# itmo153277/JoshUpscale

Hardware: AMD Instinct MI355X
Metric: frames/sec 480x270->1920x1080 recurrent SR (higher is better)
Workload: dtype bf16

## Files before the change

### joshupscale_amd/csrc/c_api.cpp

```cpp

#include "joshupscale_amd.h"
#ifdef JU_TEST_HOOKS
#include "joshupscale_amd_test.h"
#endif

#include <cstdio>
#include <cstring>
#include <fstream>
#include <ios>
#include <new>
#include <stdexcept>
#include <string>
#include <vector>

#include "engine.h"
#include "fp8.h"
#include "graphics.h"
#include "log.h"
#include "model.h"
#include "tiled.h"

struct ju_runtime {
	std::unique_ptr<ju::Engine> engine;
};
// ... 707 lines not shown
		if (key == nullptr || value == nullptr) throw std::invalid_argument("ju_get_stat: null argument");
#ifndef JU_TEST_HOOKS
		if (std::strcmp(key, "scene_detector_runs") == 0) throw std::invalid_argument("unknown stat scene_detector_runs");
#endif
		*value = engineOf(const_cast<ju_runtime *>(runtime)).stat(key);
	});
}

#ifdef JU_TEST_HOOKS
int ju_debug_set(const char *key, int value) {
	return guarded([&] {
		const std::string k = key ? key : "";
		if (k == "tower_variant") ju::setTowerVariant(value);
		else if (k == "resident_fault") ju::setResidentFault(value);
		else if (k == "tower_fast") ju::setResidentTowerFast(value);
		else if (k == "res_block_plain") ju::setResBlockPlain(value);
		else if (k == "fp8_block_form") ju::setFp8BlockForm(value);
		else if (k == "pass_rerun") ju::setPassRerun(value);
		else if (k == "step_rerun") ju::setStepRerun(value);
		else if (k == "group_rerun") ju::setGroupRerun(value);
		else throw std::invalid_argument("unknown debug key " + k);
	});
}

namespace {
struct ConversionHook {
	const char *name, *family;
	bool (*admits)(const ju::YuvFormatInfo &);
	int ops;
	bool rowStrides;
// ... 524 lines not shown
```

### joshupscale_amd/csrc/engine.cpp

```cpp
#include "engine.h"

#include <cstdio>

#include <algorithm>
#include <atomic>
#include <cstdlib>
#include <cstring>
#include <memory>
#include <mutex>
#include <sstream>
#include <stdexcept>

#include "dev_switch.h"
#include "fp8.h"
#include "graphics.h"
#include "log.h"

namespace ju {

namespace {
thread_local int g_DryLaunches = 0;
}
bool launchesAreDry() { return g_DryLaunches > 0; }
DryLaunchScope::DryLaunchScope() { ++g_DryLaunches; }
// ... 1651 lines not shown

double Engine::stat(const std::string &key) const {
	if (key == "graph_replays") return static_cast<double>(m_GraphReplays);
	if (key == "eager_runs") return static_cast<double>(m_EagerRuns);
	if (key == "graph_captures") return static_cast<double>(m_InlineCaptures);
	if (key == "prepared_captures") return static_cast<double>(m_PreparedCaptures);
	if (key == "registered_pairs") return static_cast<double>(m_RegisteredPairs.size());
	if (key == "recurrent") return m_Config.recurrent() ? 1.0 : 0.0;
	if (key == "output_select") return static_cast<double>(m_Config.outputSelect);
	if (key == "resident_tower") return m_Resident ? 1.0 : 0.0;
	if (key == "resident_flow") return m_ResidentFlow ? 1.0 : 0.0;
	if (key == "tower_fast") {
		return (m_Resident && !m_Fp8Tower && residentTowerFast() && !m_Calibrate &&
		        residentTowerFastGeometry(m_Config.frameHeight, m_Config.frameWidth, m_ResGX, m_ResGY, m_ResRH)) ? 1.0 : 0.0;
	}
	if (key == "fallbacks") return static_cast<double>(m_Fallbacks);
	if (key == "lookahead_frames") return static_cast<double>(m_BatchFrames);
	if (key == "lookahead_host_frames") return static_cast<double>(m_BatchHostFrames);
	if (key == "hbd_from_state") return m_HbdFromState ? 1.0 : 0.0;
	if (key == "lookahead_yuv_frames") return static_cast<double>(m_BatchYuvFrames);
	if (key == "lookahead_max") return static_cast<double>(m_BatchMax);
	if (key == "source_scaled") return m_SrcScale.set() ? 1.0 : 0.0;
	if (key == "output_scaled") return m_OutScale.set() ? 1.0 : 0.0;
	if (key == "source_filter") return static_cast<double>(m_SrcScale.filter());
	if (key == "output_filter") return static_cast<double>(m_OutScale.filter());
	if (key == "source_mask") return m_MaskW != 0 ? 1.0 : 0.0;
	if (key == "source_stage_frames") return static_cast<double>(m_SourceFrames);
	if (key == "group_frames") return static_cast<double>(m_GroupFrames);
	if (key == "group_yuv_frames") return static_cast<double>(m_GroupYuvFrames);
	if (key == "scene_group") return m_SceneGroup ? 1.0 : 0.0;
// ... 30 lines not shown
```

### joshupscale_amd/csrc/kernels.h

```cpp
#pragma once

#include <hip/hip_runtime_api.h>

#include <cstddef>
#include <cstdint>
#include <mutex>
#include <stdexcept>
#include <string>
#include <vector>

#include "tile_geometry.h"

namespace ju {

enum DType : int { kF16 = 0, kBF16 = 1 };

inline std::size_t dtypeSize(DType) { return 2; }

class PlanLog {
public:
	void note(const std::string &line) {
		std::lock_guard<std::mutex> lock(m_Mutex);
		for (const std::string &l : m_Lines) {
			if (l == line) return;
// ... 182 lines not shown
	const std::uint8_t *frame;
	std::ptrdiff_t frameStride;
	void *state;
	std::uint8_t *outU8;
	std::ptrdiff_t outStride;
	const unsigned *sums;
};
bool residentTowerGeometry(int H, int W, int numCUs, int *GX, int *GY, int *RH);
std::size_t residentMailboxBytes(int GX, int GY, bool leaky = false);
bool residentTowerFastGeometry(int H, int W, int GX, int GY, int RH);
void setResBlockPlain(int on);
bool resBlockPlain();
void setResidentTowerFast(int on);
void setFp8BlockForm(int form);
bool residentTowerFast();
inline std::size_t residentCounterBytes(int GX, int GY) {
	return (static_cast<std::size_t>(GX) * GY * 2 * sizeof(unsigned) + 63) / 64 * 64;
}
void launchResidentTower(DType dt, const ResidentTowerParams &p, hipStream_t stream);

bool residentTowerM16();
void setTowerVariant(int variant);
int towerVariant();
void setResidentFault(int n);
int residentFaultForTests();

struct ResidentTower8Params {
	const void *in;
	void *out;
	const void *weights;
// ... 346 lines not shown
```

### joshupscale_amd/csrc/tower_kernels.hip

```cpp
#include "kernel_common.h"

namespace ju {

namespace {

constexpr int kTowerThreads = 256;
constexpr int kTowerWBytes = 9 * 64 * 64 * 2;
constexpr int kTowerTileBytes = 10 * 34 * 128;
constexpr int kTowerLds = kTowerWBytes + 2 * kTowerTileBytes;

__device__ __forceinline__ void glds16(const void *g, void *l) {
	__builtin_amdgcn_global_load_lds((const __attribute__((address_space(1))) void *)g,
	    (__attribute__((address_space(3))) void *)l, 16, 0, 0);
}

struct TowerParams {
	const void *in;
	const void *wgt;
	const float *bias;
	const void *res;
	void *out;
	int H, W, pitch;
	int tilesX, numTiles;
	int relu;
// ... 291 lines not shown
	if (rwv != 32) return false;
#endif
	const int np2 = rhv >> 1;
	for (int par = 0; par < 2; ++par) {
		const int first = par ? 1 : 2;
		int n = 0;
		for (int k = 0; k < 2; ++k) {
			const int u = first + 2 * k;
			if (u < np2 && 2 * u + 3 <= rhv) n = k + 1;
		}
		const int mine = (np2 - par + 1) >> 1;
		if (n != 2 || (mine != 3 && mine != 4)) return false;
	}
	return true;
}

struct ResidentParams {
	const void *in;
	int inPitch;
	int hasHead;
	void *out;
	const void *weights;
	const float *bias;
	uint4 *mail;
	unsigned *count;
	unsigned *error;
	unsigned long long *debug;
	int H, W, pitch;
	int GX, GY, RH;
	int nLayers;
// ... 2 lines not shown
	const float *tailB1;
	const void *tailW2;
	const float *tailB2;
	const std::uint8_t *frame;
	std::ptrdiff_t frameStride;
	void *state;
	std::uint8_t *outU8;
	std::ptrdiff_t outStride;
	const unsigned *sums;
};

typedef unsigned long long u64;
typedef __attribute__((address_space(1))) u64 gu64;
typedef __attribute__((address_space(1))) unsigned gu32;

template <typename T, int VARIANT, bool HEAD, bool TAIL = false, bool LEAKY = false, bool FAST = false>
__global__ __launch_bounds__(256, 1) void tower_resident_kernel(ResidentParams p) {
	static_assert(!FAST || ((VARIANT == 0 || VARIANT == 4) && (JU_FAST_PRERUN == 2 || JU_FAST_PRERUN == 3)), "the fast schedule is built for the product only");
	extern __shared__ __attribute__((aligned(16))) unsigned char smem[];
	constexpr bool kNoMfma = VARIANT == 2 || VARIANT == 3;
#ifdef JU_NOXCHG_DEV
	constexpr bool xchg = false;
#else
	constexpr bool xchg = !(VARIANT == 1 || VARIANT == 3);
#endif
	const int tid = threadIdx.x;
	const int wave = tid >> 6;
	const int lane = tid & 63;
	const int px = lane & 31;
	const int hh = lane >> 5;
	const int ch = wave & 1;
	const int rp = wave >> 1;
	int region;
// ... 123 lines not shown
			__builtin_amdgcn_sched_barrier(0);
			u64 t;
			asm volatile("s_memtime %0\n\ts_waitcnt lgkmcnt(0)" : "=s"(t)::"memory");
			__builtin_amdgcn_sched_barrier(0);
			return t;
		} else {
			return 0;
		}
	};
	constexpr int kOrder[12] = {4, 5, 6, 7, 0, 1, 2, 3, 8, 9, 10, 11};
	constexpr bool kPlain = VARIANT == 8;
	constexpr int kPreRun = kPlain ? 0 : FAST ? JU_FAST_PRERUN : JU_PRERUN;
	constexpr int kPreBefore = kPlain ? 0 : JU_PREBEFORE;
	TowerAcc accPre0[2], accPre1[2], accPre2[2];
	static_assert(kPreRun >= 0 && kPreRun <= 3, "at most three interior units per wave");
	Vec8<T> fb[2][4];
	auto issue = [&](unsigned rowAddr, int m, int set, int j) __attribute__((always_inline)) {
#if JU_TOWER_M16
		const int dx = m >> 2, ks32 = (m >> 1) & 1, ph = m & 1;
		const unsigned a = rowAddr + colBase[dx] + (((unsigned)(ks32 * 4 + (lane >> 4)) ^ colSwz[dx]) << 4);
		if (ph) {
			if (j == 0) asm volatile("ds_read_b128 %0, %1 offset:2048" : "=v"(fb[set][0]) : "v"(a));
			else if (j == 1) asm volatile("ds_read_b128 %0, %1 offset:6400" : "=v"(fb[set][1]) : "v"(a));
			else if (j == 2) asm volatile("ds_read_b128 %0, %1 offset:10752" : "=v"(fb[set][2]) : "v"(a));
			else asm volatile("ds_read_b128 %0, %1 offset:15104" : "=v"(fb[set][3]) : "v"(a));
			return;
		}
#else
		const int dx = m >> 2, ks = m & 3;
		const unsigned a = rowAddr + colBase[dx] + (((unsigned)(ks * 2 + hh) ^ colSwz[dx]) << 4);
#endif
		if (j == 0) asm volatile("ds_read_b128 %0, %1" : "=v"(fb[set][0]) : "v"(a));
		else if (j == 1) asm volatile("ds_read_b128 %0, %1 offset:4352" : "=v"(fb[set][1]) : "v"(a));
		else if (j == 2) asm volatile("ds_read_b128 %0, %1 offset:8704" : "=v"(fb[set][2]) : "v"(a));
		else asm volatile("ds_read_b128 %0, %1 offset:13056" : "=v"(fb[set][3]) : "v"(a));
	};
	const int np2 = rhv >> 1;
	const bool mySingle = (rhv & 1) && rp == (np2 & 1);
	const int preFirst = rp ? 1 : 2;
	int nPre = 0;
#pragma unroll
	for (int k = 0; k < kPreRun; ++k) {
		const int u = preFirst + 2 * k;
		if (u < np2 && 2 * u + 3 <= rhv) nPre = k + 1;
	}
	if constexpr (FAST && kPreRun == 3) {
		const int mine = (np2 - rp + 1) >> 1;
		nPre = nPre < mine - 1 ? nPre : mine - 1;
	}
	const int preEnd = preFirst + 2 * nPre;
	auto isPre = [&](int u) __attribute__((always_inline)) { return u >= preFirst && u < preEnd; };
	auto nextWhole = [&](int u) __attribute__((always_inline)) {
		int v = u + 2;
		if (isPre(v)) v = preEnd;
		return v < np2 ? v : -1;
	};
	const int firstWhole = isPre(rp) ? (preEnd < np2 ? preEnd : -1) : (rp < np2 ? rp : -1);
	const bool streamsInUnit = (firstWhole >= 0 || mySingle) && !kNoMfma && !kPlain;
	constexpr bool kDefer = FAST;
	const bool deferShape = residentFastShape(rhv, rwv);
	if constexpr (FAST) {
		if (!deferShape) {
			if (tid == 0) __hip_atomic_store((gu32 *)p.error, 0x6f0u, __ATOMIC_RELAXED, __HIP_MEMORY_SCOPE_SYSTEM);
			return;
		}
	}

#if JU_TOWER_M16
	const bool validLo = (lane & 15) < rwv, validHi = 16 + (lane & 15) < rwv;
	auto groupValid = [&](const int g) __attribute__((always_inline)) { return FAST || ((g >> 1) ? validHi : validLo); };
#else
	const bool lanesValid = px < rwv;
	auto groupValid = [&](const int) __attribute__((always_inline)) { return lanesValid; };
#endif
	typedef unsigned u32x4 __attribute__((ext_vector_type(4)));
	const __amdgpu_buffer_rsrc_t mailRsrc = __builtin_amdgcn_make_buffer_rsrc(
	    (void *)p.mail, 0, (int)((size_t)p.GX * p.GY * 2 * (LEAKY ? 2 : 1) * kResMailSlots * 16), 0x00020000);
	constexpr int kSc1 = 16;
	Vec4<T> rvNext[2][4];
	auto epiValue = [&](auto resTag, const TowerAcc &a, const int g, const Vec4<T> &rv, float(&v)[4]) __attribute__((always_inline)) {
#pragma unroll
		for (int i = 0; i < 4; ++i) v[i] = accElem(a, 4 * g + i);
		if constexpr (decltype(resTag)::value) {
#pragma unroll
			for (int i = 0; i < 4; ++i) v[i] += static_cast<float>(rv[i]);
		}
		if constexpr (VARIANT == 5 && !LEAKY) {
			if (groupValid(g)) {
#pragma unroll
				for (int i = 0; i < 4; ++i) calibMax = fmaxf(calibMax, v[i]);
			}
		}
	};
	auto epiStore = [&](auto outTag, const int row, const int g, float(&v)[4]) __attribute__((always_inline)) {
		constexpr int outOff = decltype(outTag)::value;
		if constexpr (LEAKY) {
#pragma unroll
			for (int i = 0; i < 4; ++i) v[i] = fmaxf(v[i], v[i] * p.slope);
			if constexpr (VARIANT == 5) {
#pragma unroll
				for (int i = 0; i < 4; ++i) calibMax = fmaxf(calibMax, fabsf(v[i]));
			}
			*reinterpret_cast<Vec4<T> *>(smem + outOff + row * kResRowBytes + outsw[g]) = pack4<T>(v[0], v[1], v[2], v[3]);
		} else {
			*reinterpret_cast<Vec4<T> *>(smem + outOff + row * kResRowBytes + outsw[g]) =
			    reluPacked<T>(pack4<T>(v[0], v[1], v[2], v[3]));
		}
	};
	auto unitSeg = [&](auto rowsTag, auto kindTag, auto resTag, auto inTag, auto outTag, TowerAcc(&acc)[2],
	                   const int layer, const int unit, const bool primed, const int nextUnit,
	                   const bool nextFinish, auto streamTag, auto defTag, TowerAcc(&dacc)[2], const int dunit,
	                   auto epiTag) __attribute__((always_inline)) {
		constexpr bool streamNext = decltype(streamTag)::value;
		constexpr bool DEF = decltype(defTag)::value;
		constexpr bool EPI = decltype(epiTag)::value;
		constexpr int ROWS = decltype(rowsTag)::value;
		constexpr int KIND = decltype(kindTag)::value;
		constexpr bool residual = decltype(resTag)::value;
		constexpr int inOff = decltype(inTag)::value;
		constexpr int outOff = decltype(outTag)::value;
		constexpr int P0 = KIND == 1 ? 4 : 0;
		constexpr int P1 = KIND == 0 ? 4 : 12;
		const u64 tu0 = stamp();
		constexpr int NR = ROWS + 2;
		constexpr int NM = 3 * ROWS;
		const int ra = 1 + 2 * unit;
		if constexpr (KIND != 1 && kNoMfma) {
#pragma unroll
			for (int r = 0; r < ROWS; ++r) acc[r] = biasVec;
		}
		unsigned rowAddr = ldsBase + inOff + (2 * unit) * kResRowBytes;
		asm volatile("" : "+v"(rowAddr));
		constexpr bool kFetchRes = !EPI && residual && KIND != 0;
		const int dra = 1 + 2 * dunit;
		const TowerAcc dacc0 = dacc[0], dacc1 = dacc[1];
		float dv[4];
		unsigned dlo = 0, dhi = 0;
		auto defSlot = [&](const int pos, const int k, const int part = -1) __attribute__((always_inline)) {
					if constexpr (DEF) {
						const int j = pos - P0;
						if (j < 8) {
							const int r = j >> 2, g = j & 3;
							if (k < 5 && part == 1) {
							} else if (k < 4) {
								dv[k] = accElem(r ? dacc1 : dacc0, 4 * g + k);
								if constexpr (residual) {
									dv[k] += static_cast<float>(rvNext[r][g][k]);
									asm volatile("" : "+v"(dv[k]));
								}
								if constexpr (LEAKY) {
									const float t = dv[k] * p.slope;
									asm volatile("v_max_f32 %0, %1, %2" : "=v"(dv[k]) : "v"(dv[k]), "v"(t));
								}
							} else if (k == 4) {
								const Vec4<T> pk = pack4<T>(dv[0], dv[1], dv[2], dv[3]);
								typedef unsigned u32x2d __attribute__((ext_vector_type(2)));
								const u32x2d w = __builtin_bit_cast(u32x2d, pk);
								dlo = w[0];
								dhi = w[1];
								asm volatile("" : "+v"(dlo), "+v"(dhi));
							} else {
								typedef unsigned u32x2d __attribute__((ext_vector_type(2)));
								if (part != 1) {
									const Vec4<T> pk = __builtin_bit_cast(Vec4<T>, u32x2d{dlo, dhi});
									const u32x2d w = __builtin_bit_cast(u32x2d, LEAKY ? pk : reluPacked<T>(pk));
									dlo = w[0];
									dhi = w[1];
									if (part == 0) asm volatile("" : "+v"(dlo), "+v"(dhi));
								}
								if (part != 0) {
									const Vec4<T> o = __builtin_bit_cast(Vec4<T>, u32x2d{dlo, dhi});
									if (groupValid(g)) *reinterpret_cast<Vec4<T> *>(smem + outOff + (dra + r) * kResRowBytes + outsw[g]) = o;
								}
							}
						}
					}
		};
		if (!kNoMfma) {
			if (!primed) {
				asm volatile("s_waitcnt lgkmcnt(0)" ::: "memory");
				__builtin_amdgcn_sched_barrier(0);
#pragma unroll
				for (int j = 0; j < NR; ++j) issue(rowAddr, kOrder[P0], 0, j);
			}
#pragma unroll
			for (int pos = P0; pos < P1; ++pos) {
				const int m = kOrder[pos];
				const int set = (pos - P0) & 1;
				const bool more = (pos + 1 < P1);
				const int dx = m >> 2;
				[[maybe_unused]] const int ks = m & 3;
#pragma unroll
				for (int k = 0; k < NM; ++k) {
					const int dy = ROWS == 2 ? (k >> 1) : k;
					const int r = ROWS == 2 ? (k & 1) : 0;
					const int need = r + dy;
					const bool fresh = ROWS == 2 ? (k == 0 || k == 1 || k == 3 || k == 5) : true;
					if (fresh) {
						const int issuedNext = more ? (k < NR ? k : NR) : 0;
						const int younger = (DEF && pos > P0 && pos - P0 <= 8 ? 1 : 0) +
						                    (kFetchRes && pos == P1 - 1 ? 2 * (k < 4 ? k : 4) : 0);
						const int allowed = (NR - 1 - need) + issuedNext + younger;
						if (allowed >= 12) asm volatile("s_waitcnt lgkmcnt(12)" ::: "memory");
						else if (allowed == 11) asm volatile("s_waitcnt lgkmcnt(11)" ::: "memory");
						else if (allowed == 10) asm volatile("s_waitcnt lgkmcnt(10)" ::: "memory");
						else if (allowed == 9) asm volatile("s_waitcnt lgkmcnt(9)" ::: "memory");
						else if (allowed == 8) asm volatile("s_waitcnt lgkmcnt(8)" ::: "memory");
						else if (allowed == 7) asm volatile("s_waitcnt lgkmcnt(7)" ::: "memory");
						else if (allowed == 6) asm volatile("s_waitcnt lgkmcnt(6)" ::: "memory");
						else if (allowed == 5) asm volatile("s_waitcnt lgkmcnt(5)" ::: "memory");
						else if (allowed == 4) asm volatile("s_waitcnt lgkmcnt(4)" ::: "memory");
						else if (allowed == 3) asm volatile("s_waitcnt lgkmcnt(3)" ::: "memory");
						else if (allowed == 2) asm volatile("s_waitcnt lgkmcnt(2)" ::: "memory");
						else if (allowed == 1) asm volatile("s_waitcnt lgkmcnt(1)" ::: "memory");
						else asm volatile("s_waitcnt lgkmcnt(0)" ::: "memory");
						__builtin_amdgcn_sched_barrier(0);
					}
#if JU_TOWER_M16
					{
						const int ks32 = (m >> 1) & 1, ph = m & 1;
						const bool first = KIND != 1 && (pos == P0 || pos == P0 + 1) && dy == 0;
#pragma unroll
						for (int c16 = 0; c16 < 2; ++c16) {
							const int kf = ks32 * 2 + c16, sl = ph * 2 + c16;
							acc[r].q[sl] = mfma16(dx == 1 ? wm[dy * 4 + kf] : ws[dy * 8 + (dx >> 1) * 4 + kf], fb[set][need],
							    first ? biasVec.q[sl] : acc[r].q[sl]);
							if (c16 == 0) {
								defSlot(pos, k, 0);
								__builtin_amdgcn_sched_barrier(0);
							}
						}
						defSlot(pos, k, 1);
						if constexpr (KIND == 2) {
							if (streamNext && (m & 1) && (ROWS == 2 ? (k & 1) : true)) {
								const int sdy = ROWS == 2 ? (k >> 1) : k;
#pragma unroll
								for (int c16 = 0; c16 < 2; ++c16) {
									const int kf = ks32 * 2 + c16;
									const Vec8<T> nf = loadWeightFrag(layer + 1, (sdy * 3 + dx) * 4 + kf);
									if (dx == 1) wm[sdy * 4 + kf] = nf;
									else ws[sdy * 8 + (dx >> 1) * 4 + kf] = nf;
								}
							}
						}
					}
#else
					acc[r] = mfma32(dx == 1 ? wm[dy * 4 + ks] : ws[dy * 8 + (dx >> 1) * 4 + ks], fb[set][need],
					    (KIND != 1 && pos == P0 && dy == 0) ? biasVec : acc[r]);
#endif
					if (more && k < NR) issue(rowAddr, kOrder[pos + 1 < 12 ? pos + 1 : 11], set ^ 1, k);
#if !JU_TOWER_M16
					defSlot(pos, k);
#endif
					if constexpr (kFetchRes) {
						if (pos == P1 - 1 && k < 4) {
							const int ra0 = 1 + 2 * unit;
							rvNext[(2 * k) >> 2][(2 * k) & 3] = *reinterpret_cast<const Vec4<T> *>(
							    smem + outOff + (ra0 + ((2 * k) >> 2)) * kResRowBytes + outsw[(2 * k) & 3]);
							rvNext[(2 * k + 1) >> 2][(2 * k + 1) & 3] = *reinterpret_cast<const Vec4<T> *>(
							    smem + outOff + (ra0 + ((2 * k + 1) >> 2)) * kResRowBytes + outsw[(2 * k + 1) & 3]);
						}
					}
					__builtin_amdgcn_sched_barrier(0);
				}
				if constexpr (KIND == 2) {
					if (streamNext) {
#if JU_TOWER_M16
						if (pos == 1) loadBias(layer + 1);
#else
						if (pos == 0) loadBias(layer + 1);
// ... 2 lines not shown
#else
#pragma unroll
						for (int dy = 0; dy < 3; ++dy) {
							const Vec8<T> nf = loadWeightFrag(layer + 1, (dy * 3 + dx) * 4 + ks);
							if (dx == 1) wm[dy * 4 + ks] = nf;
							else ws[dy * 8 + (dx >> 1) * 4 + ks] = nf;
						}
#endif
						__builtin_amdgcn_sched_barrier(0);
					}
				}
			}
			if (nextUnit >= 0) {
				const unsigned na = ldsBase + inOff + (2 * nextUnit) * kResRowBytes;
				const bool nextSingle = (nextUnit == np2);
				if (nextFinish) {
#pragma unroll
					for (int j = 0; j < 4; ++j) issue(na, kOrder[4], 0, j);
				} else {
#pragma unroll
					for (int j = 0; j < 3; ++j) issue(na, kOrder[0], 0, j);
					if (!nextSingle) issue(na, kOrder[0], 0, 3);
				}
				__builtin_amdgcn_sched_barrier(0);
			}
		}
		const u64 tu1 = stamp();
		if constexpr (KIND == 0) prof[7] += tu1 - tu0;
#ifdef JU_TOWER_SEGPROF
		else if constexpr (KIND == 1 && !DEF) prof[3] += tu1 - tu0;
		else if constexpr (KIND == 1 && DEF) prof[4] += tu1 - tu0;
		else if constexpr (KIND == 2 && !streamNext) prof[5] += tu1 - tu0;
		else prof[6] += tu1 - tu0;
#else
		else prof[5] += tu1 - tu0;
#endif
		if constexpr (KIND != 0 && EPI) {
			{
				Vec4<T> rv[ROWS][4];
				if (residual) {
#pragma unroll
					for (int r = 0; r < ROWS; ++r) {
#pragma unroll
						for (int g = 0; g < 4; ++g) {
							rv[r][g] = *reinterpret_cast<const Vec4<T> *>(
							    smem + outOff + (ra + r) * kResRowBytes + outsw[g]);
						}
					}
					asm volatile("s_waitcnt lgkmcnt(0)" ::: "memory");
				}
#pragma unroll
				for (int r = 0; r < ROWS; ++r) {
// ... 4 lines not shown
						if (groupValid(g)) epiStore(outTag, ra + r, g, v);
					}
				}
			}
			const u64 tu2 = stamp();
#ifndef JU_TOWER_SEGPROF
			prof[6] += tu2 - tu1;
#endif
		}
	};
	using R2 = std::integral_constant<int, 2>;
	using R1 = std::integral_constant<int, 1>;
	using KPre = std::integral_constant<int, 0>;
	using KFin = std::integral_constant<int, 1>;
	using KWhole = std::integral_constant<int, 2>;
	auto preRun = [&](auto inTag, auto outTag, auto loTag, auto hiTag, const int layer, const bool primedFirst)
	                  __attribute__((always_inline)) {
		constexpr int LO = decltype(loTag)::value, HI = decltype(hiTag)::value;
		auto slot = [&](TowerAcc(&acc)[2], const int k) __attribute__((always_inline)) {
			if (k < nPre) {
				const int nu = (k + 1 < kPreRun && k + 1 < nPre) ? preFirst + 2 * (k + 1) : -1;
				unitSeg(R2{}, KPre{}, std::false_type{}, inTag, outTag, acc, layer, preFirst + 2 * k,
				    (k > 0 || primedFirst) && !kNoMfma, nu, false, std::false_type{}, std::false_type{}, acc, 0, std::true_type{});
			}
		};
		if constexpr (LO <= 0 && 0 < HI) slot(accPre0, 0);
		if constexpr (LO <= 1 && 1 < HI) slot(accPre1, 1);
		if constexpr (LO <= 2 && 2 < HI) slot(accPre2, 2);
	};
	auto finishLayer = [&](auto resTag, auto inTag, auto outTag, const int layer, const bool streamW) __attribute__((always_inline)) {
		const int afterPre = firstWhole >= 0 ? firstWhole : (mySingle ? np2 : -1);
		if constexpr (kDefer) {
			{
				using Y = std::true_type;
				using N = std::false_type;
				const int ua = firstWhole, ub = nextWhole(firstWhole);
				int lastUnit = ua;
				unitSeg(R2{}, KFin{}, resTag, inTag, outTag, accPre0, layer, preFirst, false, preFirst + 2, true, N{}, N{}, accPre0, 0, N{});
				if (kPreRun == 3 && nPre == 3) {
					unitSeg(R2{}, KFin{}, resTag, inTag, outTag, accPre1, layer, preFirst + 2, true, preFirst + 4, true, N{}, Y{}, accPre0, preFirst, N{});
					unitSeg(R2{}, KFin{}, resTag, inTag, outTag, accPre2, layer, preFirst + 4, true, ua, false, N{}, Y{}, accPre1, preFirst + 2, N{});
					if (streamW) unitSeg(R2{}, KWhole{}, resTag, inTag, outTag, accPre0, layer, ua, true, -1, false, Y{}, Y{}, accPre2, preFirst + 4, N{});
					else unitSeg(R2{}, KWhole{}, resTag, inTag, outTag, accPre0, layer, ua, true, -1, false, N{}, Y{}, accPre2, preFirst + 4, N{});
				} else {
					unitSeg(R2{}, KFin{}, resTag, inTag, outTag, accPre1, layer, preFirst + 2, true, ua, false, N{}, Y{}, accPre0, preFirst, N{});
					if (ub >= 0) {
						unitSeg(R2{}, KWhole{}, resTag, inTag, outTag, accPre2, layer, ua, true, ub, false, N{}, Y{}, accPre1, preFirst + 2, N{});
// ... 310 lines not shown
		if constexpr (VARIANT == 5) {
			float m = calibMax;
#pragma unroll
			for (int off = 32; off > 0; off >>= 1) m = fmaxf(m, __shfl_xor(m, off));
			if (lane == 0) atomicMax(reinterpret_cast<unsigned *>(p.debug) + i, __float_as_uint(m));
			calibMax = 0.f;
		}
		const u64 t1 = stamp();
		__syncthreads();
		const u64 t2 = stamp();
		if (more && xchg) publish(OutT{}, i);
		const bool primePre = more && nPre > 0 && !kNoMfma;
		if (primePre) {
			const unsigned na = ldsBase + OutT::value + (2 * preFirst) * kResRowBytes;
#pragma unroll
			for (int j = 0; j < 4; ++j) issue(na, kOrder[0], 0, j);
			__builtin_amdgcn_sched_barrier(0);
		}
		const u64 t3 = stamp();
		if (more && !streamsInUnit) {
			loadBias(i + 1);
			loadMidWeights(i + 1);
			loadSideWeights(i + 1);
		}
		const u64 t4 = stamp();
		if (more && xchg) {
			using Z = std::integral_constant<int, 0>;
			using Split = std::integral_constant<int, kPreBefore>;
			using N = std::integral_constant<int, kPreRun>;
			preRun(OutT{}, InT{}, Z{}, Split{}, i + 1, primePre);
			const bool okFill = fillHalo(OutT{}, i, [&]() __attribute__((always_inline)) {
// ... 85 lines not shown
		for (int i = tid; i < rhv * kResRW * 8; i += 256) {
			const int c = i & 7;
			const int pxl = (i >> 3) % kResRW;
			const int row = (i >> 3) / kResRW;
			if (pxl < rwv) {
				const int rr = row + 1, cc = pxl + 1;
				const uint4 v = *reinterpret_cast<const uint4 *>(
				    smem + finalOff + rr * kResRowBytes + cc * 128 + ((c ^ ((cc >> 1) & 7)) << 4));
				*reinterpret_cast<uint4 *>(
				    out + ((size_t)(y0 + rr) * p.pitch + x0 + cc) * 64 + c * 8) = v;
			}
		}
	}
}

template <typename T, int VARIANT, bool HEAD, bool TAIL = false, bool LEAKY = false, bool FAST = false>
void launchResidentT(const ResidentParams &p, hipStream_t stream) {
	auto kern = tower_resident_kernel<T, VARIANT, HEAD, TAIL, LEAKY, FAST>;
	static std::atomic<std::uint64_t> ldsDone{0};
	ensureDynamicLds(reinterpret_cast<const void *>(kern), kResLds, &ldsDone, "resident tower");
	const int grid = p.GX * p.GY - (g_ResidentFault < p.GX * p.GY ? g_ResidentFault : 0);
	hipLaunchKernelGGL(kern, dim3(grid), dim3(256), kResLds, stream, p);
	hipCheckLaunch("tower_resident");
}

}

void launchConvTower(DType dt, const ConvParams &p, hipStream_t stream) {
	const int pitch = towerPitch(p.W);
	const bool fits = p.taps == 9 && p.cin == 64 && p.cout == 64 && !p.outHead && p.nb == 2 &&
	                  p.inPitch == pitch && p.outPitch == pitch &&
	                  (p.res == nullptr || p.resPitch == pitch);
	if (!fits) {
// ... 24 lines not shown

bool residentTowerGeometry(int H, int W, int numCUs, int *GX, int *GY, int *RH) {
	const int gx = (W + kResRW - 1) / kResRW;
	const int gy = (H + kResMaxRH - 1) / kResMaxRH;
	if (gx * gy > numCUs) return false;
	*GX = gx;
	*GY = gy;
	*RH = (H + gy - 1) / gy;
	return true;
}

bool residentTowerFastGeometry(int H, int W, int GX, int GY, int RH) {
	const int lastH = H - (GY - 1) * RH, lastW = W - (GX - 1) * kResRW;
	return residentFastShape(RH, kResRW) && residentFastShape(lastH, kResRW) && residentFastShape(RH, lastW) &&
	       residentFastShape(lastH, lastW);
}

std::size_t residentMailboxBytes(int GX, int GY, bool leaky) {
	return static_cast<std::size_t>(GX) * GY * 2 * kResMailSlots * 16 * (leaky ? 2 : 1);
}

void launchResidentTower(DType dt, const ResidentTowerParams &q, hipStream_t stream) {
	ResidentParams p{};
	const std::size_t origin = towerOrigin(q.W) * 64 * 2;
	p.in = q.in;
	p.inPitch = q.inPitch ? q.inPitch : q.W;
	p.hasHead = q.hasHead;
	p.out = static_cast<unsigned char *>(q.out) - origin;
	p.weights = q.weights;
	p.bias = q.bias;
// ... 11 lines not shown
	p.slope = q.slope;
	p.tailW1 = q.tailW1;
	p.tailB1 = q.tailB1;
	p.tailW2 = q.tailW2;
	p.tailB2 = q.tailB2;
	p.frame = q.frame;
	p.frameStride = q.frameStride;
	p.state = q.state;
	p.outU8 = q.outU8;
	p.outStride = q.outStride;
	p.sums = q.sums;
	if ((p.nLayers & 1) != (p.hasHead ? 1 : 0)) {
		throw std::invalid_argument("resident tower: layer count must be 2*blocks (+1 with a head)");
	}
	const bool fast = residentTowerFast() && residentTowerFastGeometry(p.H, p.W, p.GX, p.GY, p.RH);
#ifdef JU_TOWER_DEV
	if (q.leaky || dt == kF16 || !p.hasHead) throw std::invalid_argument("resident tower: developer build");
	if (p.tailW1 != nullptr) {
		if (fast) launchResidentT<bf16, 0, true, true, false, true>(p, stream);
		else launchResidentT<bf16, 0, true, true>(p, stream);
	} else if (g_TowerVariant == 8) launchResidentT<bf16, 8, true>(p, stream);
	else if (g_TowerVariant == 4) {
		if (fast) launchResidentT<bf16, 4, true, false, false, true>(p, stream);
		else launchResidentT<bf16, 4, true>(p, stream);
	} else if (fast) launchResidentT<bf16, 0, true, false, false, true>(p, stream);
	else launchResidentT<bf16, 0, true>(p, stream);
	return;
#else
	if (q.leaky) {
		if (!(q.slope >= 0.0f && q.slope <= 1.0f)) throw std::invalid_argument("resident tower: negative slope outside [0, 1]");
		if (p.tailW1 != nullptr) throw std::invalid_argument("resident tower: the fused tail is built for ReLU models");
		if (!p.hasHead) {
			if (fast) {
				if (dt == kF16) launchResidentT<f16, 0, false, false, true, true>(p, stream);
				else launchResidentT<bf16, 0, false, false, true, true>(p, stream);
			} else {
				if (dt == kF16) launchResidentT<f16, 0, false, false, true>(p, stream);
				else launchResidentT<bf16, 0, false, false, true>(p, stream);
			}
		} else if (g_TowerVariant == 8) {
// ... 10 lines not shown
			else launchResidentT<bf16, 0, true, false, true>(p, stream);
		}
		return;
	}
	if (!p.hasHead) {
		if (fast) {
			if (dt == kF16) launchResidentT<f16, 0, false, false, false, true>(p, stream);
			else launchResidentT<bf16, 0, false, false, false, true>(p, stream);
		} else {
			if (dt == kF16) launchResidentT<f16, 0, false>(p, stream);
			else launchResidentT<bf16, 0, false>(p, stream);
		}
		return;
	}
	if (p.tailW1 != nullptr) {
		if (fast) {
			if (dt == kF16) launchResidentT<f16, 0, true, true, false, true>(p, stream);
			else launchResidentT<bf16, 0, true, true, false, true>(p, stream);
		} else {
			if (dt == kF16) launchResidentT<f16, 0, true, true>(p, stream);
			else launchResidentT<bf16, 0, true, true>(p, stream);
		}
		return;
	}
	if (dt == kF16) {
		if (g_TowerVariant == 8) launchResidentT<f16, 8, true>(p, stream);
		else if (fast) launchResidentT<f16, 0, true, false, false, true>(p, stream);
		else launchResidentT<f16, 0, true>(p, stream);
		return;
	}
	switch (g_TowerVariant) {
	case 8: launchResidentT<bf16, 8, true>(p, stream); break;
	case 1: launchResidentT<bf16, 1, true>(p, stream); break;
	case 2: launchResidentT<bf16, 2, true>(p, stream); break;
	case 3: launchResidentT<bf16, 3, true>(p, stream); break;
	case 4:
		if (fast) launchResidentT<bf16, 4, true, false, false, true>(p, stream);
		else launchResidentT<bf16, 4, true>(p, stream);
		break;
	case 5:
		(void)hipMemsetAsync(p.debug, 0, static_cast<std::size_t>(p.nLayers) * sizeof(unsigned), stream);
		launchResidentT<bf16, 5, true>(p, stream);
		break;
	default:
		if (fast) launchResidentT<bf16, 0, true, false, false, true>(p, stream);
		else launchResidentT<bf16, 0, true>(p, stream);
		break;
	}
#endif
}


}
```

Baseline: 2214.

## Process four output rows per unit in the fast resident tower schedule

Adds a UROWS=4 form of the resident tower kernel, where each MFMA unit computes four output rows instead of two. Each LDS input row fragment is then reused across more rows, and there are fewer unit segments per layer. The pre-run, finish and whole-unit segments, the deferred epilogue slots and the LDS-wait accounting are reworked for quads. It becomes the default when the tile geometry gives 14- or 16-row by 32-column tiles. In exchange it holds more accumulators and fragment registers, with extra register pressure and more complex scheduling.

Result: faster. 2246 (median of 6 runs) (+1.5%).

```diff
diff --git a/joshupscale_amd/csrc/c_api.cpp b/joshupscale_amd/csrc/c_api.cpp
--- a/joshupscale_amd/csrc/c_api.cpp
+++ b/joshupscale_amd/csrc/c_api.cpp
@@ -745,6 +745,7 @@
 		if (k == "tower_variant") ju::setTowerVariant(value);
 		else if (k == "resident_fault") ju::setResidentFault(value);
 		else if (k == "tower_fast") ju::setResidentTowerFast(value);
+		else if (k == "tower_unit_rows") ju::setResidentTowerUnitRows(value);
 		else if (k == "res_block_plain") ju::setResBlockPlain(value);
 		else if (k == "fp8_block_form") ju::setFp8BlockForm(value);
 		else if (k == "pass_rerun") ju::setPassRerun(value);
diff --git a/joshupscale_amd/csrc/engine.cpp b/joshupscale_amd/csrc/engine.cpp
--- a/joshupscale_amd/csrc/engine.cpp
+++ b/joshupscale_amd/csrc/engine.cpp
@@ -1689,6 +1689,10 @@
 		return (m_Resident && !m_Fp8Tower && residentTowerFast() && !m_Calibrate &&
 		        residentTowerFastGeometry(m_Config.frameHeight, m_Config.frameWidth, m_ResGX, m_ResGY, m_ResRH)) ? 1.0 : 0.0;
 	}
+	if (key == "tower_unit_rows") {
+		const bool fast = stat("tower_fast") != 0.0;
+		return (fast && m_Config.genActivation != 1) ? static_cast<double>(residentTowerUnitRows(m_Config.frameHeight, m_Config.frameWidth, m_ResGX, m_ResGY, m_ResRH)) : 2.0;
+	}
 	if (key == "fallbacks") return static_cast<double>(m_Fallbacks);
 	if (key == "lookahead_frames") return static_cast<double>(m_BatchFrames);
 	if (key == "lookahead_host_frames") return static_cast<double>(m_BatchHostFrames);
diff --git a/joshupscale_amd/csrc/kernels.h b/joshupscale_amd/csrc/kernels.h
--- a/joshupscale_amd/csrc/kernels.h
+++ b/joshupscale_amd/csrc/kernels.h
@@ -220,6 +220,8 @@
 void setResidentTowerFast(int on);
 void setFp8BlockForm(int form);
 bool residentTowerFast();
+int residentTowerUnitRows(int H, int W, int GX, int GY, int RH);
+void setResidentTowerUnitRows(int rows);
 inline std::size_t residentCounterBytes(int GX, int GY) {
 	return (static_cast<std::size_t>(GX) * GY * 2 * sizeof(unsigned) + 63) / 64 * 64;
 }
diff --git a/joshupscale_amd/csrc/tower_kernels.hip b/joshupscale_amd/csrc/tower_kernels.hip
--- a/joshupscale_amd/csrc/tower_kernels.hip
+++ b/joshupscale_amd/csrc/tower_kernels.hip
@@ -329,6 +329,8 @@
 	}
 	return true;
 }
+
+__host__ __device__ inline bool residentFastQuadShape(int rhv, int rwv) { return rwv == 32 && (rhv == 16 || rhv == 14); }
 
 struct ResidentParams {
 	const void *in;
@@ -361,9 +363,11 @@
 typedef __attribute__((address_space(1))) u64 gu64;
 typedef __attribute__((address_space(1))) unsigned gu32;
 
-template <typename T, int VARIANT, bool HEAD, bool TAIL = false, bool LEAKY = false, bool FAST = false>
+template <typename T, int VARIANT, bool HEAD, bool TAIL = false, bool LEAKY = false, bool FAST = false, int UROWS = 2>
 __global__ __launch_bounds__(256, 1) void tower_resident_kernel(ResidentParams p) {
 	static_assert(!FAST || ((VARIANT == 0 || VARIANT == 4) && (JU_FAST_PRERUN == 2 || JU_FAST_PRERUN == 3)), "the fast schedule is built for the product only");
+	static_assert(UROWS == 2 || (UROWS == 4 && FAST && !LEAKY && JU_TOWER_M16 && JU_FAST_PRERUN == 2 && JU_PREBEFORE == 1),
+	    "row quads are a form of the ReLU fast schedule in the 16x16x32 shape");
 	extern __shared__ __attribute__((aligned(16))) unsigned char smem[];
 	constexpr bool kNoMfma = VARIANT == 2 || VARIANT == 3;
 #ifdef JU_NOXCHG_DEV
@@ -517,7 +521,8 @@
 	constexpr int kPreBefore = kPlain ? 0 : JU_PREBEFORE;
 	TowerAcc accPre0[2], accPre1[2], accPre2[2];
 	static_assert(kPreRun >= 0 && kPreRun <= 3, "at most three interior units per wave");
-	Vec8<T> fb[2][4];
+	TowerAcc accQ0[4], accQ1[4];
+	Vec8<T> fb[2][UROWS + 2];
 	auto issue = [&](unsigned rowAddr, int m, int set, int j) __attribute__((always_inline)) {
 #if JU_TOWER_M16
 		const int dx = m >> 2, ks32 = (m >> 1) & 1, ph = m & 1;
@@ -526,7 +531,11 @@
 			if (j == 0) asm volatile("ds_read_b128 %0, %1 offset:2048" : "=v"(fb[set][0]) : "v"(a));
 			else if (j == 1) asm volatile("ds_read_b128 %0, %1 offset:6400" : "=v"(fb[set][1]) : "v"(a));
 			else if (j == 2) asm volatile("ds_read_b128 %0, %1 offset:10752" : "=v"(fb[set][2]) : "v"(a));
-			else asm volatile("ds_read_b128 %0, %1 offset:15104" : "=v"(fb[set][3]) : "v"(a));
+			else if (j == 3) asm volatile("ds_read_b128 %0, %1 offset:15104" : "=v"(fb[set][3]) : "v"(a));
+			else if constexpr (UROWS == 4) {
+				if (j == 4) asm volatile("ds_read_b128 %0, %1 offset:19456" : "=v"(fb[set][4]) : "v"(a));
+				else asm volatile("ds_read_b128 %0, %1 offset:23808" : "=v"(fb[set][5]) : "v"(a));
+			}
 			return;
 		}
 #else
@@ -536,17 +545,22 @@
 		if (j == 0) asm volatile("ds_read_b128 %0, %1" : "=v"(fb[set][0]) : "v"(a));
 		else if (j == 1) asm volatile("ds_read_b128 %0, %1 offset:4352" : "=v"(fb[set][1]) : "v"(a));
 		else if (j == 2) asm volatile("ds_read_b128 %0, %1 offset:8704" : "=v"(fb[set][2]) : "v"(a));
-		else asm volatile("ds_read_b128 %0, %1 offset:13056" : "=v"(fb[set][3]) : "v"(a));
+		else if (j == 3) asm volatile("ds_read_b128 %0, %1 offset:13056" : "=v"(fb[set][3]) : "v"(a));
+		else if constexpr (UROWS == 4) {
+			if (j == 4) asm volatile("ds_read_b128 %0, %1 offset:17408" : "=v"(fb[set][4]) : "v"(a));
+			else asm volatile("ds_read_b128 %0, %1 offset:21760" : "=v"(fb[set][5]) : "v"(a));
+		}
 	};
 	const int np2 = rhv >> 1;
 	const bool mySingle = (rhv & 1) && rp == (np2 & 1);
-	const int preFirst = rp ? 1 : 2;
+	const int preFirst = UROWS == 4 ? (rp ? 2 : 4) : (rp ? 1 : 2);
 	int nPre = 0;
 #pragma unroll
 	for (int k = 0; k < kPreRun; ++k) {
 		const int u = preFirst + 2 * k;
 		if (u < np2 && 2 * u + 3 <= rhv) nPre = k + 1;
 	}
+	if constexpr (UROWS == 4) nPre = 1;
 	if constexpr (FAST && kPreRun == 3) {
 		const int mine = (np2 - rp + 1) >> 1;
 		nPre = nPre < mine - 1 ? nPre : mine - 1;
@@ -559,9 +573,9 @@
 		return v < np2 ? v : -1;
 	};
 	const int firstWhole = isPre(rp) ? (preEnd < np2 ? preEnd : -1) : (rp < np2 ? rp : -1);
-	const bool streamsInUnit = (firstWhole >= 0 || mySingle) && !kNoMfma && !kPlain;
+	const bool streamsInUnit = UROWS == 4 || ((firstWhole >= 0 || mySingle) && !kNoMfma && !kPlain);
 	constexpr bool kDefer = FAST;
-	const bool deferShape = residentFastShape(rhv, rwv);
+	const bool deferShape = UROWS == 4 ? residentFastQuadShape(rhv, rwv) : residentFastShape(rhv, rwv);
 	if constexpr (FAST) {
 		if (!deferShape) {
 			if (tid == 0) __hip_atomic_store((gu32 *)p.error, 0x6f0u, __ATOMIC_RELAXED, __HIP_MEMORY_SCOPE_SYSTEM);
@@ -580,7 +594,7 @@
 	const __amdgpu_buffer_rsrc_t mailRsrc = __builtin_amdgcn_make_buffer_rsrc(
 	    (void *)p.mail, 0, (int)((size_t)p.GX * p.GY * 2 * (LEAKY ? 2 : 1) * kResMailSlots * 16), 0x00020000);
 	constexpr int kSc1 = 16;
-	Vec4<T> rvNext[2][4];
+	Vec4<T> rvNext[UROWS][4];
 	auto epiValue = [&](auto resTag, const TowerAcc &a, const int g, const Vec4<T> &rv, float(&v)[4]) __attribute__((always_inline)) {
 #pragma unroll
 		for (int i = 0; i < 4; ++i) v[i] = accElem(a, 4 * g + i);
@@ -610,10 +624,10 @@
 			    reluPacked<T>(pack4<T>(v[0], v[1], v[2], v[3]));
 		}
 	};
-	auto unitSeg = [&](auto rowsTag, auto kindTag, auto resTag, auto inTag, auto outTag, TowerAcc(&acc)[2],
+	auto unitSeg = [&](auto rowsTag, auto kindTag, auto resTag, auto inTag, auto outTag, auto &acc,
 	                   const int layer, const int unit, const bool primed, const int nextUnit,
-	                   const bool nextFinish, auto streamTag, auto defTag, TowerAcc(&dacc)[2], const int dunit,
-	                   auto epiTag) __attribute__((always_inline)) {
+	                   const bool nextFinish, auto streamTag, auto defTag, auto &dacc, const int dunit,
+	                   auto epiTag, const int nextPos = -1, const int nextNR = 4) __attribute__((always_inline)) {
 		constexpr bool streamNext = decltype(streamTag)::value;
 		constexpr bool DEF = decltype(defTag)::value;
 		constexpr bool EPI = decltype(epiTag)::value;
@@ -622,59 +636,64 @@
 		constexpr bool residual = decltype(resTag)::value;
 		constexpr int inOff = decltype(inTag)::value;
 		constexpr int outOff = decltype(outTag)::value;
-		constexpr int P0 = KIND == 1 ? 4 : 0;
-		constexpr int P1 = KIND == 0 ? 4 : 12;
+		constexpr bool kPreKind = KIND == 0 || KIND == 3;
+		constexpr int P0 = KIND == 1 ? 4 : KIND == 3 ? 2 : 0;
+		constexpr int P1 = KIND == 0 ? (ROWS == 4 ? 2 : 4) : KIND == 3 ? 4 : 12;
+		static_assert(KIND != 3 || ROWS == 4, "only a quad's pre-run is split");
 		const u64 tu0 = stamp();
 		constexpr int NR = ROWS + 2;
 		constexpr int NM = 3 * ROWS;
 		const int ra = 1 + 2 * unit;
-		if constexpr (KIND != 1 && kNoMfma) {
+		if constexpr ((KIND == 0 || KIND == 2) && kNoMfma) {
 #pragma unroll
 			for (int r = 0; r < ROWS; ++r) acc[r] = biasVec;
 		}
 		unsigned rowAddr = ldsBase + inOff + (2 * unit) * kResRowBytes;
 		asm volatile("" : "+v"(rowAddr));
-		constexpr bool kFetchRes = !EPI && residual && KIND != 0;
+		constexpr bool kFetchRes = !EPI && residual && !kPreKind;
 		const int dra = 1 + 2 * dunit;
 		const TowerAcc dacc0 = dacc[0], dacc1 = dacc[1];
+		const TowerAcc dacc2 = dacc[ROWS == 4 ? 2 : 0], dacc3 = dacc[ROWS == 4 ? 3 : 1];
 		float dv[4];
 		unsigned dlo = 0, dhi = 0;
 		auto defSlot = [&](const int pos, const int k, const int part = -1) __attribute__((always_inline)) {
 					if constexpr (DEF) {
 						const int j = pos - P0;
 						if (j < 8) {
-							const int r = j >> 2, g = j & 3;
-							if (k < 5 && part == 1) {
-							} else if (k < 4) {
-								dv[k] = accElem(r ? dacc1 : dacc0, 4 * g + k);
-								if constexpr (residual) {
-									dv[k] += static_cast<float>(rvNext[r][g][k]);
-									asm volatile("" : "+v"(dv[k]));
-								}
-								if constexpr (LEAKY) {
-									const float t = dv[k] * p.slope;
-									asm volatile("v_max_f32 %0, %1, %2" : "=v"(dv[k]) : "v"(dv[k]), "v"(t));
-								}
-							} else if (k == 4) {
-								const Vec4<T> pk = pack4<T>(dv[0], dv[1], dv[2], dv[3]);
-								typedef unsigned u32x2d __attribute__((ext_vector_type(2)));
-								const u32x2d w = __builtin_bit_cast(u32x2d, pk);
-								dlo = w[0];
-								dhi = w[1];
-								asm volatile("" : "+v"(dlo), "+v"(dhi));
-							} else {
-								typedef unsigned u32x2d __attribute__((ext_vector_type(2)));
-								if (part != 1) {
+							const int kk = ROWS == 4 ? k % 6 : k;
+							const int gi = ROWS == 4 ? 2 * j + k / 6 : j;
+							const int r = gi >> 2, g = gi & 3;
+							typedef unsigned u32x2d __attribute__((ext_vector_type(2)));
+							if (part != 1) {
+								if (kk < 4) {
+									dv[kk] = accElem(r == 0 ? dacc0 : r == 1 ? dacc1 : r == 2 ? dacc2 : dacc3, 4 * g + kk);
+									if constexpr (residual) {
+										dv[kk] += static_cast<float>(rvNext[r][g][kk]);
+										asm volatile("" : "+v"(dv[kk]));
+									}
+									if constexpr (LEAKY) {
+										const float t = dv[kk] * p.slope;
+										asm volatile("v_max_f32 %0, %1, %2" : "=v"(dv[kk]) : "v"(dv[kk]), "v"(t));
+									}
+								} else if (kk == 4) {
+									const Vec4<T> pk = pack4<T>(dv[0], dv[1], dv[2], dv[3]);
+									const u32x2d w = __builtin_bit_cast(u32x2d, pk);
+									dlo = w[0];
+									dhi = w[1];
+									asm volatile("" : "+v"(dlo), "+v"(dhi));
+								} else {
 									const Vec4<T> pk = __builtin_bit_cast(Vec4<T>, u32x2d{dlo, dhi});
 									const u32x2d w = __builtin_bit_cast(u32x2d, LEAKY ? pk : reluPacked<T>(pk));
 									dlo = w[0];
 									dhi = w[1];
 									if (part == 0) asm volatile("" : "+v"(dlo), "+v"(dhi));
 								}
-								if (part != 0) {
-									const Vec4<T> o = __builtin_bit_cast(Vec4<T>, u32x2d{dlo, dhi});
-									if (groupValid(g)) *reinterpret_cast<Vec4<T> *>(smem + outOff + (dra + r) * kResRowBytes + outsw[g]) = o;
-								}
+							}
+							if (part != 0 && (ROWS == 4 ? (k == 6 || k == 11) : k == 5)) {
+								const int wi = (ROWS == 4 && k == 6) ? gi - 1 : gi;
+								const int wr = wi >> 2, wg = wi & 3;
+								const Vec4<T> o = __builtin_bit_cast(Vec4<T>, u32x2d{dlo, dhi});
+								if (groupValid(wg)) *reinterpret_cast<Vec4<T> *>(smem + outOff + (dra + wr) * kResRowBytes + outsw[wg]) = o;
 							}
 						}
 					}
@@ -695,14 +714,15 @@
 				[[maybe_unused]] const int ks = m & 3;
 #pragma unroll
 				for (int k = 0; k < NM; ++k) {
-					const int dy = ROWS == 2 ? (k >> 1) : k;
-					const int r = ROWS == 2 ? (k & 1) : 0;
+					const int dy = k / ROWS;
+					const int r = k % ROWS;
 					const int need = r + dy;
-					const bool fresh = ROWS == 2 ? (k == 0 || k == 1 || k == 3 || k == 5) : true;
+					const bool fresh = dy == 0 || r == ROWS - 1;
 					if (fresh) {
 						const int issuedNext = more ? (k < NR ? k : NR) : 0;
-						const int younger = (DEF && pos > P0 && pos - P0 <= 8 ? 1 : 0) +
-						                    (kFetchRes && pos == P1 - 1 ? 2 * (k < 4 ? k : 4) : 0);
+						const bool prevDef = DEF && pos > P0 && pos - P0 <= 8;
+						const int younger = (ROWS == 4 ? (prevDef ? 2 : 0) + (DEF && pos - P0 < 8 && k >= 7 ? 1 : 0) : (prevDef ? 1 : 0)) +
+						                    (kFetchRes && pos == P1 - 1 ? 2 * (k < 2 * ROWS ? k : 2 * ROWS) : 0);
 						const int allowed = (NR - 1 - need) + issuedNext + younger;
 						if (allowed >= 12) asm volatile("s_waitcnt lgkmcnt(12)" ::: "memory");
 						else if (allowed == 11) asm volatile("s_waitcnt lgkmcnt(11)" ::: "memory");
@@ -722,7 +742,7 @@
 #if JU_TOWER_M16
 					{
 						const int ks32 = (m >> 1) & 1, ph = m & 1;
-						const bool first = KIND != 1 && (pos == P0 || pos == P0 + 1) && dy == 0;
+						const bool first = pos < 2 && dy == 0;
 #pragma unroll
 						for (int c16 = 0; c16 < 2; ++c16) {
 							const int kf = ks32 * 2 + c16, sl = ph * 2 + c16;
@@ -735,8 +755,8 @@
 						}
 						defSlot(pos, k, 1);
 						if constexpr (KIND == 2) {
-							if (streamNext && (m & 1) && (ROWS == 2 ? (k & 1) : true)) {
-								const int sdy = ROWS == 2 ? (k >> 1) : k;
+							if (streamNext && (m & 1) && r == ROWS - 1) {
+								const int sdy = dy;
 #pragma unroll
 								for (int c16 = 0; c16 < 2; ++c16) {
 									const int kf = ks32 * 2 + c16;
@@ -756,7 +776,7 @@
 					defSlot(pos, k);
 #endif
 					if constexpr (kFetchRes) {
-						if (pos == P1 - 1 && k < 4) {
+						if (pos == P1 - 1 && k < 2 * ROWS) {
 							const int ra0 = 1 + 2 * unit;
 							rvNext[(2 * k) >> 2][(2 * k) & 3] = *reinterpret_cast<const Vec4<T> *>(
 							    smem + outOff + (ra0 + ((2 * k) >> 2)) * kResRowBytes + outsw[(2 * k) & 3]);
@@ -789,7 +809,13 @@
 			if (nextUnit >= 0) {
 				const unsigned na = ldsBase + inOff + (2 * nextUnit) * kResRowBytes;
 				const bool nextSingle = (nextUnit == np2);
-				if (nextFinish) {
+				if constexpr (UROWS == 4) {
+					const int npos = nextPos >= 0 ? nextPos : (nextFinish ? 4 : 0);
+#pragma unroll
+					for (int j = 0; j < 6; ++j) {
+						if (j < nextNR) issue(na, kOrder[npos], 0, j);
+					}
+				} else if (nextFinish) {
 #pragma unroll
 					for (int j = 0; j < 4; ++j) issue(na, kOrder[4], 0, j);
 				} else {
@@ -801,7 +827,7 @@
 			}
 		}
 		const u64 tu1 = stamp();
-		if constexpr (KIND == 0) prof[7] += tu1 - tu0;
+		if constexpr (kPreKind) prof[7] += tu1 - tu0;
 #ifdef JU_TOWER_SEGPROF
 		else if constexpr (KIND == 1 && !DEF) prof[3] += tu1 - tu0;
 		else if constexpr (KIND == 1 && DEF) prof[4] += tu1 - tu0;
@@ -810,7 +836,7 @@
 #else
 		else prof[5] += tu1 - tu0;
 #endif
-		if constexpr (KIND != 0 && EPI) {
+		if constexpr (!kPreKind && EPI) {
 			{
 				Vec4<T> rv[ROWS][4];
 				if (residual) {
@@ -845,9 +871,21 @@
 	using KPre = std::integral_constant<int, 0>;
 	using KFin = std::integral_constant<int, 1>;
 	using KWhole = std::integral_constant<int, 2>;
+	using R4 = std::integral_constant<int, 4>;
+	using KPre2 = std::integral_constant<int, 3>;
 	auto preRun = [&](auto inTag, auto outTag, auto loTag, auto hiTag, const int layer, const bool primedFirst)
 	                  __attribute__((always_inline)) {
 		constexpr int LO = decltype(loTag)::value, HI = decltype(hiTag)::value;
+		if constexpr (UROWS == 4) {
+			if constexpr (LO <= 0 && 0 < HI) {
+				unitSeg(R4{}, KPre{}, std::false_type{}, inTag, outTag, accQ0, layer, preFirst, primedFirst, preFirst, false,
+				    std::false_type{}, std::false_type{}, accQ0, 0, std::true_type{}, 2, 6);
+			}
+			if constexpr (LO <= 1 && 1 < HI) {
+				unitSeg(R4{}, KPre2{}, std::false_type{}, inTag, outTag, accQ0, layer, preFirst, true, -1, false,
+				    std::false_type{}, std::false_type{}, accQ0, 0, std::true_type{});
+			}
+		} else {
 		auto slot = [&](TowerAcc(&acc)[2], const int k) __attribute__((always_inline)) {
 			if (k < nPre) {
 				const int nu = (k + 1 < kPreRun && k + 1 < nPre) ? preFirst + 2 * (k + 1) : -1;
@@ -858,10 +896,41 @@
 		if constexpr (LO <= 0 && 0 < HI) slot(accPre0, 0);
 		if constexpr (LO <= 1 && 1 < HI) slot(accPre1, 1);
 		if constexpr (LO <= 2 && 2 < HI) slot(accPre2, 2);
+		}
 	};
 	auto finishLayer = [&](auto resTag, auto inTag, auto outTag, const int layer, const bool streamW) __attribute__((always_inline)) {
 		const int afterPre = firstWhole >= 0 ? firstWhole : (mySingle ? np2 : -1);
-		if constexpr (kDefer) {
+		if constexpr (UROWS == 4) {
+			using Y = std::true_type;
+			using N = std::false_type;
+			const int edge = rp ? 6 : 0;
+			if (rhv == 16 || rp == 0) {
+				unitSeg(R4{}, KFin{}, resTag, inTag, outTag, accQ0, layer, preFirst, false, edge, false, N{}, N{}, accQ0, 0, N{}, 0, 6);
+				if (streamW) unitSeg(R4{}, KWhole{}, resTag, inTag, outTag, accQ1, layer, edge, true, -1, false, Y{}, Y{}, accQ0, preFirst, N{});
+				else unitSeg(R4{}, KWhole{}, resTag, inTag, outTag, accQ1, layer, edge, true, -1, false, N{}, Y{}, accQ0, preFirst, N{});
+				const u64 te0 = stamp();
+				const int ra = 1 + 2 * edge;
+#pragma unroll
+				for (int r = 0; r < 4; ++r) {
+#pragma unroll
+					for (int g = 0; g < 4; ++g) {
+						float v[4];
+						epiValue(resTag, accQ1[r], g, rvNext[r][g], v);
+						epiStore(outTag, ra + r, g, v);
+					}
+				}
+#ifndef JU_TOWER_SEGPROF
+				prof[6] += stamp() - te0;
+#else
+				(void)te0;
+#endif
+			} else {
+				TowerAcc accPair[2];
+				unitSeg(R4{}, KFin{}, resTag, inTag, outTag, accQ0, layer, preFirst, false, edge, false, N{}, N{}, accQ0, 0, Y{}, 0, 4);
+				if (streamW) unitSeg(R2{}, KWhole{}, resTag, inTag, outTag, accPair, layer, edge, true, -1, false, Y{}, N{}, accPair, 0, Y{});
+				else unitSeg(R2{}, KWhole{}, resTag, inTag, outTag, accPair, layer, edge, true, -1, false, N{}, N{}, accPair, 0, Y{});
+			}
+		} else if constexpr (kDefer) {
 			{
 				using Y = std::true_type;
 				using N = std::false_type;
@@ -1202,7 +1271,7 @@
 		if (primePre) {
 			const unsigned na = ldsBase + OutT::value + (2 * preFirst) * kResRowBytes;
 #pragma unroll
-			for (int j = 0; j < 4; ++j) issue(na, kOrder[0], 0, j);
+			for (int j = 0; j < UROWS + 2; ++j) issue(na, kOrder[0], 0, j);
 			__builtin_amdgcn_sched_barrier(0);
 		}
 		const u64 t3 = stamp();
@@ -1318,9 +1387,9 @@
 	}
 }
 
-template <typename T, int VARIANT, bool HEAD, bool TAIL = false, bool LEAKY = false, bool FAST = false>
+template <typename T, int VARIANT, bool HEAD, bool TAIL = false, bool LEAKY = false, bool FAST = false, int UROWS = 2>
 void launchResidentT(const ResidentParams &p, hipStream_t stream) {
-	auto kern = tower_resident_kernel<T, VARIANT, HEAD, TAIL, LEAKY, FAST>;
+	auto kern = tower_resident_kernel<T, VARIANT, HEAD, TAIL, LEAKY, FAST, UROWS>;
 	static std::atomic<std::uint64_t> ldsDone{0};
 	ensureDynamicLds(reinterpret_cast<const void *>(kern), kResLds, &ldsDone, "resident tower");
 	const int grid = p.GX * p.GY - (g_ResidentFault < p.GX * p.GY ? g_ResidentFault : 0);
@@ -1375,6 +1444,15 @@
 	const int lastH = H - (GY - 1) * RH, lastW = W - (GX - 1) * kResRW;
 	return residentFastShape(RH, kResRW) && residentFastShape(lastH, kResRW) && residentFastShape(RH, lastW) &&
 	       residentFastShape(lastH, lastW);
+}
+
+static std::atomic<int> g_TowerUnitRows{4};
+void setResidentTowerUnitRows(int rows) { g_TowerUnitRows = rows == 2 ? 2 : 4; }
+int residentTowerUnitRows(int H, int W, int GX, int GY, int RH) {
+	const int lastH = H - (GY - 1) * RH, lastW = W - (GX - 1) * kResRW;
+	const bool quads = JU_TOWER_M16 != 0 && residentFastQuadShape(RH, kResRW) && residentFastQuadShape(lastH, kResRW) &&
+	                   residentFastQuadShape(RH, lastW) && residentFastQuadShape(lastH, lastW);
+	return quads && g_TowerUnitRows.load() == 4 ? 4 : 2;
 }
 
 std::size_t residentMailboxBytes(int GX, int GY, bool leaky) {
@@ -1416,16 +1494,20 @@
 		throw std::invalid_argument("resident tower: layer count must be 2*blocks (+1 with a head)");
 	}
 	const bool fast = residentTowerFast() && residentTowerFastGeometry(p.H, p.W, p.GX, p.GY, p.RH);
+	const bool quad = fast && !q.leaky && residentTowerUnitRows(p.H, p.W, p.GX, p.GY, p.RH) == 4;
 #ifdef JU_TOWER_DEV
 	if (q.leaky || dt == kF16 || !p.hasHead) throw std::invalid_argument("resident tower: developer build");
 	if (p.tailW1 != nullptr) {
-		if (fast) launchResidentT<bf16, 0, true, true, false, true>(p, stream);
+		if (quad) launchResidentT<bf16, 0, true, true, false, true, 4>(p, stream);
+		else if (fast) launchResidentT<bf16, 0, true, true, false, true>(p, stream);
 		else launchResidentT<bf16, 0, true, true>(p, stream);
 	} else if (g_TowerVariant == 8) launchResidentT<bf16, 8, true>(p, stream);
 	else if (g_TowerVariant == 4) {
-		if (fast) launchResidentT<bf16, 4, true, false, false, true>(p, stream);
+		if (quad) launchResidentT<bf16, 4, true, false, false, true, 4>(p, stream);
+		else if (fast) launchResidentT<bf16, 4, true, false, false, true>(p, stream);
 		else launchResidentT<bf16, 4, true>(p, stream);
-	} else if (fast) launchResidentT<bf16, 0, true, false, false, true>(p, stream);
+	} else if (quad) launchResidentT<bf16, 0, true, false, false, true, 4>(p, stream);
+	else if (fast) launchResidentT<bf16, 0, true, false, false, true>(p, stream);
 	else launchResidentT<bf16, 0, true>(p, stream);
 	return;
 #else
@@ -1466,7 +1548,10 @@
 		return;
 	}
 	if (p.tailW1 != nullptr) {
-		if (fast) {
+		if (quad) {
+			if (dt == kF16) launchResidentT<f16, 0, true, true, false, true, 4>(p, stream);
+			else launchResidentT<bf16, 0, true, true, false, true, 4>(p, stream);
+		} else if (fast) {
 			if (dt == kF16) launchResidentT<f16, 0, true, true, false, true>(p, stream);
 			else launchResidentT<bf16, 0, true, true, false, true>(p, stream);
 		} else {
@@ -1477,6 +1562,7 @@
 	}
 	if (dt == kF16) {
 		if (g_TowerVariant == 8) launchResidentT<f16, 8, true>(p, stream);
+		else if (quad) launchResidentT<f16, 0, true, false, false, true, 4>(p, stream);
 		else if (fast) launchResidentT<f16, 0, true, false, false, true>(p, stream);
 		else launchResidentT<f16, 0, true>(p, stream);
 		return;
@@ -1487,7 +1573,8 @@
 	case 2: launchResidentT<bf16, 2, true>(p, stream); break;
 	case 3: launchResidentT<bf16, 3, true>(p, stream); break;
 	case 4:
-		if (fast) launchResidentT<bf16, 4, true, false, false, true>(p, stream);
+		if (quad) launchResidentT<bf16, 4, true, false, false, true, 4>(p, stream);
+		else if (fast) launchResidentT<bf16, 4, true, false, false, true>(p, stream);
 		else launchResidentT<bf16, 4, true>(p, stream);
 		break;
 	case 5:
@@ -1495,7 +1582,8 @@
 		launchResidentT<bf16, 5, true>(p, stream);
 		break;
 	default:
-		if (fast) launchResidentT<bf16, 0, true, false, false, true>(p, stream);
+		if (quad) launchResidentT<bf16, 0, true, false, false, true, 4>(p, stream);
+		else if (fast) launchResidentT<bf16, 0, true, false, false, true>(p, stream);
 		else launchResidentT<bf16, 0, true>(p, stream);
 		break;
 	}
```
